# hamaadshah/gan_deeplearning4j

Hardware: NVIDIA H100
Metric: images/sec (full G+D step) (higher is better)
Workload: dtype bf16

## Files before the change

### gan_deeplearning4j_b200/csrc/kernels_ew.cu

```cuda
#include <stdlib.h>
#include <algorithm>
#include "kernels.h"
#include "common.cuh"

namespace b2g {

uint64_t g_launch_count = 0;
const char* g_ew_last_kernel = "";

template <typename T>
__global__ void nchw_f32_to_nhwc_kernel(const float* __restrict__ src, T* __restrict__ dst, int N, int C, int HW) { pdl_enter();
  size_t total = (size_t)N * C * HW;
  for (size_t i = blockIdx.x * (size_t)blockDim.x + threadIdx.x; i < total; i += (size_t)gridDim.x * blockDim.x) {
    int c = i % C; size_t t = i / C; int p = t % HW; size_t n = t / HW;
    stf(dst, i, src[(n * C + c) * HW + p]);
  }
}
template <typename T>
__global__ void nhwc_to_nchw_f32_kernel(const T* __restrict__ src, float* __restrict__ dst, int N, int C, int HW) { pdl_enter();
  size_t total = (size_t)N * C * HW;
  for (size_t i = blockIdx.x * (size_t)blockDim.x + threadIdx.x; i < total; i += (size_t)gridDim.x * blockDim.x) {
    int p = i % HW; size_t t = i / HW; int c = t % C; size_t n = t / C;
    dst[i] = ldf(src, (n * HW + p) * C + c);
  }
}
template <typename T>
__global__ void permute_kernel(const T* __restrict__ src, T* __restrict__ dst, int N, int C, int HW, int to_nhwc) { pdl_enter();
  size_t total = (size_t)N * C * HW;
  for (size_t i = blockIdx.x * (size_t)blockDim.x + threadIdx.x; i < total; i += (size_t)gridDim.x * blockDim.x) {
    if (to_nhwc) { int c = i % C; size_t t = i / C; int p = t % HW; size_t n = t / HW; dst[i] = src[(n * C + c) * HW + p]; }
    else         { int p = i % HW; size_t t = i / HW; int c = t % C; size_t n = t / C; dst[i] = src[(n * HW + p) * C + c]; }
  }
}
#define DISPATCH_ACT(act, ACTC, ...)                                                            \
  switch (act) {                                                                                \
    case ACT_IDENTITY: { constexpr int ACTC = ACT_IDENTITY; __VA_ARGS__; } break;               \
    case ACT_RELU: { constexpr int ACTC = ACT_RELU; __VA_ARGS__; } break;                       \
    case ACT_LRELU: { constexpr int ACTC = ACT_LRELU; __VA_ARGS__; } break;                     \
    default: { constexpr int ACTC = -1; __VA_ARGS__; } break;                                   \
  }
int device_sm_count() {
  static int sms[64] = {}; int d = 0; cudaGetDevice(&d); if (d < 0 || d >= 64) d = 0;
  if (!sms[d]) { int v = 0; cudaDeviceGetAttribute(&v, cudaDevAttrMultiProcessorCount, d); sms[d] = v > 0 ? v : 1; }
  return sms[d];
}
static inline int vec4_blocks(size_t n_vec) { const size_t cap = (size_t)device_sm_count() * 4; size_t b = (n_vec + 1023) / 1024; if (b > cap) b = cap; if (b < 1) b = 1; return (int)b; }
static inline int ew_blocks(size_t n, int per = 256) { const size_t cap = (size_t)device_sm_count() * 16; size_t b = (n + per - 1) / per; if (b > cap) b = cap; if (b < 1) b = 1; return (int)b; }

void k_nchw_f32_to_nhwc(int prec, const float* src, void* dst, int N, int C, int HW, cudaStream_t s) {
  size_t n = (size_t)N * C * HW; if (!n) return;
  DISPATCH_PREC(prec, T, (launch_pdl(nchw_f32_to_nhwc_kernel<T>, dim3(ew_blocks(n)), dim3(256), (size_t)(0), s, src, (T*)dst, N, C, HW))); LAUNCHED();
}
void k_nhwc_to_nchw_f32(int prec, const void* src, float* dst, int N, int C, int HW, cudaStream_t s) {
  size_t n = (size_t)N * C * HW; if (!n) return;
  DISPATCH_PREC(prec, T, (launch_pdl(nhwc_to_nchw_f32_kernel<T>, dim3(ew_blocks(n)), dim3(256), (size_t)(0), s, (const T*)src, dst, N, C, HW))); LAUNCHED();
}
void k_permute(int prec, const void* src, void* dst, int N, int C, int HW, int to_nhwc, cudaStream_t s) {
  size_t n = (size_t)N * C * HW; if (!n) return;
  DISPATCH_PREC(prec, T, (launch_pdl(permute_kernel<T>, dim3(ew_blocks(n)), dim3(256), (size_t)(0), s, (const T*)src, (T*)dst, N, C, HW, to_nhwc))); LAUNCHED();
}
__global__ void cast_f32_to_bf16_kernel(const float* __restrict__ src, __nv_bfloat16* __restrict__ dst, size_t n) { pdl_enter();
  for (size_t i = blockIdx.x * (size_t)blockDim.x + threadIdx.x; i < n; i += (size_t)gridDim.x * blockDim.x) dst[i] = __float2bfloat16_rn(src[i]);
}
void k_cast_f32_to_bf16(const float* src, __nv_bfloat16* dst, size_t n, cudaStream_t s) {
  if (!n) return; launch_pdl(cast_f32_to_bf16_kernel, dim3(ew_blocks(n)), dim3(256), (size_t)(0), s, src, dst, n); LAUNCHED();
}
static const int SLICE_ELEMS = 1 << 20;
static inline int pick_slices(int rows, int C) {
  int cap = SLICE_ELEMS / (C > 0 ? C : 1); if (cap < 1) cap = 1; if (cap > 2048) cap = 2048;
  int S = rows / 8; if (S < 1) S = 1; if (S > cap) S = cap; return S;
}
size_t k_bn_scratch_floats(int C, int groups) { return (size_t)2 * groups * (SLICE_ELEMS + 2 * (size_t)C) + 64; }
size_t k_colsum_scratch_floats(int C) { return (size_t)(SLICE_ELEMS + C) + 64; }

__device__ __forceinline__ void unpack8(const uint4& u, float (&v)[8]) {
  const __nv_bfloat162* h = reinterpret_cast<const __nv_bfloat162*>(&u);
#pragma unroll
  for (int j = 0; j < 4; ++j) { float2 f = __bfloat1622float2(h[j]); v[2 * j] = f.x; v[2 * j + 1] = f.y; }
}
__device__ __forceinline__ uint4 pack8(const float (&v)[8]) {
  uint4 u; __nv_bfloat162* h = reinterpret_cast<__nv_bfloat162*>(&u);
#pragma unroll
  for (int j = 0; j < 4; ++j) h[j] = __floats2bfloat162_rn(v[2 * j], v[2 * j + 1]);
  return u;
}

template <typename T>
__global__ void bn_stats_partial_kernel(const T* __restrict__ x, int rows, int C, int S, float* __restrict__ psum, float* __restrict__ psq, float* __restrict__ pivot) { pdl_enter();
  int g = blockIdx.y;
  int idx = blockIdx.x * blockDim.x + threadIdx.x;
  if (idx >= S * C) return;
  int c = idx % C, sl = idx / C;
  const T* xg = x + (size_t)g * rows * C;
  const float k = ldf(xg, c);
  if (sl == 0) pivot[g * C + c] = k;
  float a = 0.f, b = 0.f;
  for (int r = sl; r < rows; r += S) { float v = ldf(xg, (size_t)r * C + c) - k; a += v; b = fmaf(v, v, b); }
  psum[((size_t)g * S + sl) * C + c] = a; psq[((size_t)g * S + sl) * C + c] = b;
}
static inline int vec_ty(int C) { int c8 = C / 8; int ty = 256 / c8; return ty < 1 ? 1 : ty; }
static inline bool vec_ok(int prec, int C) { return prec == PREC_BF16 && C % 8 == 0 && C / 8 <= 256 && 256 % (C / 8) == 0; }
static inline int vec_blocks(int rows, int C) { int ty = vec_ty(C); int b = rows / (ty * 4); int cap = SLICE_ELEMS / C; if (cap > 256) cap = 256; if (b > cap) b = cap; if (b < 1) b = 1; return b; }
template <int NV>
__device__ __forceinline__ void block_fold_write(float (&acc)[NV][8], int C, int C8, int c8, int ty, int TY, float* const (&dst)[NV], size_t row_off) {
  __shared__ float sred[NV][2048];
#pragma unroll
  for (int v = 0; v < NV; ++v)
#pragma unroll
    for (int j = 0; j < 8; ++j) sred[v][ty * C + c8 * 8 + j] = acc[v][j];
  __syncthreads();
  for (int c = threadIdx.x; c < C; c += blockDim.x) {
#pragma unroll
    for (int v = 0; v < NV; ++v) { float a = 0.f; for (int k = 0; k < TY; ++k) a += sred[v][k * C + c]; dst[v][row_off + c] = a; }
  }
}
__global__ void __launch_bounds__(1024) bn_stats_final_kernel(const float* __restrict__ psum, const float* __restrict__ psq, const float* __restrict__ pivot, int rows, int C, int S, int groups, float eps,
                                      float* __restrict__ mean, float* __restrict__ invstd,
                                      const float* __restrict__ run_mean, const float* __restrict__ run_var, float* g_mean, float* g_var, float decay) { pdl_enter();
  __shared__ double sa[32][33], sb[32][33];
  const int tx = threadIdx.x & 31, ty = threadIdx.x >> 5, c = blockIdx.x * 32 + tx;
  double acc_gm = 0.0, acc_gv = 0.0;
  for (int g = 0; g < groups; ++g) {
    double a = 0.0, b = 0.0;
    if (c < C) for (int sl0 = ty; sl0 < S; sl0 += 32 * 8) {
      float va[8], vb[8];
#pragma unroll
      for (int q = 0; q < 8; ++q) { const int sl = sl0 + 32 * q; va[q] = sl < S ? psum[((size_t)g * S + sl) * C + c] : 0.f; vb[q] = sl < S ? psq[((size_t)g * S + sl) * C + c] : 0.f; }
#pragma unroll
      for (int q = 0; q < 8; ++q) { a += va[q]; b += vb[q]; }
    }
    sa[ty][tx] = a; sb[ty][tx] = b;
    __syncthreads();
    if (ty == 0 && c < C) {
      for (int k = 1; k < 32; ++k) { a += sa[k][tx]; b += sb[k][tx]; }
      const double d = a / rows, mu = (double)pivot[g * C + c] + d; double var = b / rows - d * d; if (var < 0) var = 0;
      mean[g * C + c] = (float)mu; invstd[g * C + c] = (float)(1.0 / sqrt(var + (double)eps));
      if (g_mean) { acc_gm += (1.0 - decay) * ((double)run_mean[c] - mu); acc_gv += (1.0 - decay) * ((double)run_var[c] - var); }
    }
    __syncthreads();
  }
  if (g_mean && ty == 0 && c < C) { g_mean[c] = (float)(acc_gm / groups); g_var[c] = (float)(acc_gv / groups); }
}
void k_bn_stats(int prec, const void* x, int rows, int C, int groups, float* scratch, float* mean, float* invstd, float eps,
                const float* run_mean, const float* run_var, float* g_mean, float* g_var, float decay, cudaStream_t s) {
  const int S = pick_slices(rows, C);
  float* psum = scratch; float* psq = scratch + (size_t)groups * S * C; float* pivot = psq + (size_t)groups * S * C;
  dim3 grid((S * C + 255) / 256, groups);
  DISPATCH_PREC(prec, T, (launch_pdl(bn_stats_partial_kernel<T>, dim3(grid), dim3(256), (size_t)(0), s, (const T*)x, rows, C, S, psum, psq, pivot)));
  LAUNCHED();
  launch_pdl(bn_stats_final_kernel, dim3((C + 31) / 32), dim3(1024), (size_t)(0), s, psum, psq, (const float*)pivot, rows, C, S, groups, eps, mean, invstd, run_mean, run_var, g_mean, g_var, decay); LAUNCHED();
}
__global__ void bn_prep_infer_kernel(const float* __restrict__ rm, const float* __restrict__ rv, int C, int groups, float eps, float* mean, float* invstd) { pdl_enter();
  int i = blockIdx.x * blockDim.x + threadIdx.x; if (i >= C * groups) return;
  int c = i % C; mean[i] = rm[c]; invstd[i] = 1.0f / sqrtf(rv[c] + eps);
}
__global__ void bn_fold_kernel(const float* __restrict__ rm, const float* __restrict__ rv, const float* __restrict__ gamma, const float* __restrict__ beta, const float* __restrict__ cb, int C, float eps, float* scale, float* shift) { pdl_enter();
  int c = blockIdx.x * blockDim.x + threadIdx.x; if (c >= C) return;
  const float sc = gamma[c] / sqrtf(rv[c] + eps); scale[c] = sc; shift[c] = beta[c] - rm[c] * sc + (cb ? cb[c] * sc : 0.f);
}
void k_bn_fold(const float* rm, const float* rv, const float* gamma, const float* beta, const float* cb, int C, float eps, float* scale, float* shift, cudaStream_t s) {
  launch_pdl(bn_fold_kernel, dim3((C + 255) / 256), dim3(256), (size_t)0, s, rm, rv, gamma, beta, cb, C, eps, scale, shift); LAUNCHED();
}
void k_bn_prep_infer(const float* run_mean, const float* run_var, int C, int groups, float eps, float* mean, float* invstd, cudaStream_t s) {
  launch_pdl(bn_prep_infer_kernel, dim3((C * groups + 255) / 256), dim3(256), (size_t)(0), s, run_mean, run_var, C, groups, eps, mean, invstd); LAUNCHED();
}

template <typename T>
__global__ void bn_apply_kernel(const T* __restrict__ x, T* __restrict__ y, int rows, int C, int groups, const float* __restrict__ mean,
                                const float* __restrict__ invstd, const float* __restrict__ gamma, const float* __restrict__ beta, int act, float alpha) { pdl_enter();
  size_t per_group = (size_t)rows * C, total = per_group * groups;
  for (size_t i = blockIdx.x * (size_t)blockDim.x + threadIdx.x; i < total; i += (size_t)gridDim.x * blockDim.x) {
    int c = i % C; int g = i / per_group;
    float v = (ldf(x, i) - mean[g * C + c]) * invstd[g * C + c];
    stf(y, i, act_fwd(act, fmaf(gamma[c], v, beta[c]), alpha));
  }
}
template <int ACTC>
__global__ void __launch_bounds__(256, 3) bn_apply_bf16x8_kernel(const uint4* __restrict__ x, uint4* __restrict__ y, int rows, int C, int groups, const float* __restrict__ mean,
                                       const float* __restrict__ invstd, const float* __restrict__ gamma, const float* __restrict__ beta, int act, float alpha) { pdl_enter();
  const int C8 = C / 8; const size_t per_group = (size_t)rows * C8;
  const size_t t0 = blockIdx.x * (size_t)blockDim.x + threadIdx.x, stride = (size_t)gridDim.x * blockDim.x;
  const int c0 = (int)(t0 % C8) * 8;
  for (int g = 0; g < groups; ++g) {
    float mu[8], is[8], ga[8], be[8];
#pragma unroll
    for (int j = 0; j < 8; ++j) { mu[j] = mean[g * C + c0 + j]; is[j] = invstd[g * C + c0 + j]; ga[j] = gamma[c0 + j]; be[j] = beta[c0 + j]; }
    const uint4* xg = x + g * per_group; uint4* yg = y + g * per_group;
    for (size_t i = t0; i < per_group; i += 4 * stride) {
      uint4 xa[4];
#pragma unroll
      for (int q = 0; q < 4; ++q) if (i + q * stride < per_group) xa[q] = xg[i + q * stride];
#pragma unroll
      for (int q = 0; q < 4; ++q) if (i + q * stride < per_group) {
        float v[8]; unpack8(xa[q], v);
#pragma unroll
        for (int j = 0; j < 8; ++j) v[j] = act_fwd(ACTC < 0 ? act : ACTC, fmaf(ga[j], (v[j] - mu[j]) * is[j], be[j]), alpha);
        yg[i + q * stride] = pack8(v);
      }
    }
  }
}
void k_bn_apply(int prec, const void* x, void* y, int rows, int C, int groups, const float* mean, const float* invstd,
                const float* gamma, const float* beta, int act, float alpha, cudaStream_t s) {
  size_t n = (size_t)rows * C * groups; if (!n) return;
  if (vec_ok(prec, C)) {
    DISPATCH_ACT(act, ACTC, launch_pdl(bn_apply_bf16x8_kernel<ACTC>, dim3(vec4_blocks((size_t)rows * C / 8)), dim3(256), (size_t)(0), s, (const uint4*)x, (uint4*)y, rows, C, groups, mean, invstd, gamma, beta, act, alpha));
  } else {
    DISPATCH_PREC(prec, T, (launch_pdl(bn_apply_kernel<T>, dim3(ew_blocks(n)), dim3(256), (size_t)(0), s, (const T*)x, (T*)y, rows, C, groups, mean, invstd, gamma, beta, act, alpha)));
  }
  LAUNCHED();
}

template <typename T>
__global__ void bn_bwd_partial_kernel(const T* __restrict__ x, const T* __restrict__ eo, int rows, int C, int S, const float* __restrict__ mean,
                                      const float* __restrict__ invstd, const float* __restrict__ gamma, const float* __restrict__ beta, int act, float alpha,
                                      float* __restrict__ p1, float* __restrict__ p2) { pdl_enter();
  int g = blockIdx.y;
  int idx = blockIdx.x * blockDim.x + threadIdx.x;
  if (idx >= S * C) return;
  int c = idx % C, sl = idx / C;
  const T* xg = x + (size_t)g * rows * C; const T* eg = eo + (size_t)g * rows * C;
  float mu = mean[g * C + c], is = invstd[g * C + c], ga = gamma[c], be = beta[c];
  float a = 0.f, b = 0.f;
  for (int r = sl; r < rows; r += S) {
    float xh = (ldf(xg, (size_t)r * C + c) - mu) * is;
    float dy = ldf(eg, (size_t)r * C + c) * act_grad_from_pre(act, fmaf(ga, xh, be), alpha);
    a += dy; b = fmaf(dy, xh, b);
  }
  p1[((size_t)g * S + sl) * C + c] = a; p2[((size_t)g * S + sl) * C + c] = b;
}
__global__ void __launch_bounds__(1024) bn_bwd_final_kernel(const float* __restrict__ p1, const float* __restrict__ p2, int rows, int C, int S, int groups,
                                    float* __restrict__ c1, float* __restrict__ c2, float* g_gamma, float* g_beta, int want) { pdl_enter();
  __shared__ double sa[32][33], sb[32][33];
  const int tx = threadIdx.x & 31, ty = threadIdx.x >> 5, c = blockIdx.x * 32 + tx;
  double tg = 0.0, tb = 0.0;
  for (int g = 0; g < groups; ++g) {
    double a = 0.0, b = 0.0;
    if (c < C) for (int sl0 = ty; sl0 < S; sl0 += 32 * 8) {
      float va[8], vb[8];
#pragma unroll
      for (int q = 0; q < 8; ++q) { const int sl = sl0 + 32 * q; va[q] = sl < S ? p1[((size_t)g * S + sl) * C + c] : 0.f; vb[q] = sl < S ? p2[((size_t)g * S + sl) * C + c] : 0.f; }
#pragma unroll
      for (int q = 0; q < 8; ++q) { a += va[q]; b += vb[q]; }
    }
    sa[ty][tx] = a; sb[ty][tx] = b;
    __syncthreads();
    if (ty == 0 && c < C) {
      for (int k = 1; k < 32; ++k) { a += sa[k][tx]; b += sb[k][tx]; }
      c1[g * C + c] = (float)(a / rows); c2[g * C + c] = (float)(b / rows); tb += a; tg += b;
    }
    __syncthreads();
  }
  if (want && ty == 0 && c < C) { g_beta[c] += (float)tb; g_gamma[c] += (float)tg; }
}
template <typename T>
__global__ void bn_bwd_apply_kernel(const T* __restrict__ x, const T* __restrict__ eo, T* __restrict__ ei, int rows, int C, int groups,
                                    const float* __restrict__ mean, const float* __restrict__ invstd, const float* __restrict__ gamma,
                                    const float* __restrict__ beta, int act, float alpha, const float* __restrict__ c1, const float* __restrict__ c2) { pdl_enter();
  size_t per_group = (size_t)rows * C, total = per_group * groups;
  for (size_t i = blockIdx.x * (size_t)blockDim.x + threadIdx.x; i < total; i += (size_t)gridDim.x * blockDim.x) {
    int c = i % C; int g = i / per_group; int k = g * C + c;
    float xh = (ldf(x, i) - mean[k]) * invstd[k];
    float dy = ldf(eo, i) * act_grad_from_pre(act, fmaf(gamma[c], xh, beta[c]), alpha);
    stf(ei, i, gamma[c] * invstd[k] * (dy - c1[k] - xh * c2[k]));
  }
}
void k_bn_bwd(int prec, const void* x, const void* eps_out, void* eps_in, int rows, int C, int groups,
              const float* mean, const float* invstd, const float* gamma, const float* beta, int act, float alpha,
              float* scratch, float* g_gamma, float* g_beta, int want, cudaStream_t s) {
  const int S = pick_slices(rows, C);
  float* p1 = scratch; float* p2 = p1 + (size_t)groups * S * C; float* c1 = p2 + (size_t)groups * S * C; float* c2 = c1 + (size_t)groups * C;
  dim3 grid((S * C + 255) / 256, groups);
  DISPATCH_PREC(prec, T, (launch_pdl(bn_bwd_partial_kernel<T>, dim3(grid), dim3(256), (size_t)(0), s, (const T*)x, (const T*)eps_out, rows, C, S, mean, invstd, gamma, beta, act, alpha, p1, p2)));
  LAUNCHED();
  launch_pdl(bn_bwd_final_kernel, dim3((C + 31) / 32), dim3(1024), (size_t)(0), s, p1, p2, rows, C, S, groups, c1, c2, g_gamma, g_beta, want); LAUNCHED();
  if (eps_in) {
    size_t n = (size_t)rows * C * groups;
    DISPATCH_PREC(prec, T, (launch_pdl(bn_bwd_apply_kernel<T>, dim3(ew_blocks(n)), dim3(256), (size_t)(0), s, (const T*)x, (const T*)eps_out, (T*)eps_in, rows, C, groups, mean, invstd, gamma, beta, act, alpha, c1, c2)));
    LAUNCHED();
  }
}


bool k_bn_vec_ok(int prec, int C) { return vec_ok(prec, C); }
size_t k_bn_acc_elems(int C, int groups) { return (size_t)groups * 4 * C; }

template <int NV, typename A>
__device__ __forceinline__ void block_fold_acc(A (&acc)[NV][8], int C, int c8, int ty, int TY, unsigned long long* accbase ) {
  __shared__ double sred[NV][2048];
#pragma unroll
  for (int v = 0; v < NV; ++v)
#pragma unroll
    for (int j = 0; j < 8; ++j) sred[v][ty * C + c8 * 8 + j] = acc[v][j];
  __syncthreads();
  for (int c = threadIdx.x; c < C; c += blockDim.x) {
#pragma unroll
    for (int v = 0; v < NV; ++v) { double a = 0.0; for (int k = 0; k < TY; ++k) a += sred[v][k * C + c]; sacc_add(accbase + (size_t)v * 2 * C, (size_t)C, (size_t)c, a); }
  }
}
__global__ void __launch_bounds__(256) bn_stats_acc_kernel(const uint4* __restrict__ x, int rows, int C, int S, unsigned long long* __restrict__ accp) { pdl_enter();
  const int g = blockIdx.y, C8 = C / 8, TY = 256 / C8, c8 = threadIdx.x % C8, ty = threadIdx.x / C8, sl = blockIdx.x;
  const int chunk = (rows + S - 1) / S, r0 = sl * chunk, r1 = min(rows, r0 + chunk);
  const uint4* xg = x + (size_t)g * rows * C8;
  double acc[2][8];
#pragma unroll
  for (int j = 0; j < 8; ++j) { acc[0][j] = 0.0; acc[1][j] = 0.0; }
#pragma unroll 4
  for (int r = r0 + ty; r < r1; r += TY) { float v[8]; unpack8(xg[(size_t)r * C8 + c8], v);
#pragma unroll
    for (int j = 0; j < 8; ++j) { acc[0][j] += v[j]; acc[1][j] = fma((double)v[j], (double)v[j], acc[1][j]); } }
  block_fold_acc<2>(acc, C, c8, ty, TY, accp + (size_t)g * 4 * C);
}
void k_bn_stats_acc(const void* x, int rows, int C, int groups, unsigned long long* acc, cudaStream_t s) {
  const int S = vec_blocks(rows, C);
  launch_pdl(bn_stats_acc_kernel, dim3(S, groups), dim3(256), (size_t)0, s, (const uint4*)x, rows, C, S, acc); LAUNCHED();
}

__device__ __forceinline__ float bn_pre_act(int act, float x, float sc, float be, float mu) {
  return (act == ACT_RELU || act == ACT_LRELU) ? fmaf(x, sc, fmaf(-mu, sc, be)) : fmaf(x - mu, sc, be);
}
template <int ACTC>
__global__ void __launch_bounds__(256, 3) bn_apply_acc_kernel(const uint4* __restrict__ x, uint4* __restrict__ y, int rows, int C, int groups, const unsigned long long* __restrict__ accp,
                                                             const float* __restrict__ gamma, const float* __restrict__ beta, int act, float alpha, float eps, float* __restrict__ coef,
                                                             const float* __restrict__ run_mean, const float* __restrict__ run_var, float* g_mean, float* g_var, float decay, int replicas) { pdl_enter();
  extern __shared__ float s_cf[];
  const double cnt = (double)rows * replicas, inv_cnt = 1.0 / cnt;
  const bool writer = blockIdx.x == 0;
  const int C8 = C / 8; const size_t per_group = (size_t)rows * C8;
  const size_t t0 = blockIdx.x * (size_t)blockDim.x + threadIdx.x, stride = (size_t)gridDim.x * blockDim.x;
  uint4 xa[4];
#pragma unroll
  for (int q = 0; q < 4; ++q) if (t0 + q * stride < per_group) xa[q] = x[t0 + q * stride];
  for (int c = threadIdx.x; c < C; c += blockDim.x) {
    double agm = 0.0, agv = 0.0;
    for (int g = 0; g < groups; ++g) {
      const unsigned long long* a = accp + (size_t)g * 4 * C;
      const double mu = sacc_read(a, (size_t)C, (size_t)c) * inv_cnt; double var = sacc_read(a + 2 * (size_t)C, (size_t)C, (size_t)c) * inv_cnt - mu * mu; if (var < 0) var = 0;
      const float is = (float)(1.0 / sqrt(var + (double)eps)), sc = gamma[c] * is, sh = fmaf(-(float)mu, sc, beta[c]);
      s_cf[(g * 2 + 0) * C + c] = sc; s_cf[(g * 2 + 1) * C + c] = sh;
      if (writer) {
        coef[(size_t)(g * 4 + 0) * C + c] = sc; coef[(size_t)(g * 4 + 1) * C + c] = beta[c]; coef[(size_t)(g * 4 + 2) * C + c] = (float)mu; coef[(size_t)(g * 4 + 3) * C + c] = is;
        if (g_mean) { agm += (1.0 - decay) * ((double)run_mean[c] - mu); agv += (1.0 - decay) * ((double)run_var[c] - var); }
      }
    }
    if (writer && g_mean) { g_mean[c] = (float)(agm / groups); g_var[c] = (float)(agv / groups); }
  }
  __syncthreads();
  const int c0 = (int)(t0 % C8) * 8;
  bool preloaded = true;
  for (int g = 0; g < groups; ++g) {
    float sc[8], sh[8];
#pragma unroll
    for (int j = 0; j < 8; ++j) { sc[j] = s_cf[(g * 2 + 0) * C + c0 + j]; sh[j] = s_cf[(g * 2 + 1) * C + c0 + j]; }
    const uint4* xg = x + g * per_group; uint4* yg = y + g * per_group;
    for (size_t i = t0; i < per_group; i += 4 * stride) {
      if (!preloaded) {
#pragma unroll
        for (int q = 0; q < 4; ++q) if (i + q * stride < per_group) xa[q] = xg[i + q * stride];
      }
      preloaded = false;
#pragma unroll
      for (int q = 0; q < 4; ++q) if (i + q * stride < per_group) {
        float v[8]; unpack8(xa[q], v);
#pragma unroll
        for (int j = 0; j < 8; ++j) v[j] = act_fwd(ACTC < 0 ? act : ACTC, fmaf(v[j], sc[j], sh[j]), alpha);
        yg[i + q * stride] = pack8(v);
      }
    }
  }
}
void k_bn_apply_acc(const void* x, void* y, int rows, int C, int groups, const unsigned long long* acc, const float* gamma, const float* beta, int act, float alpha, float eps,
                    float* coef, const float* run_mean, const float* run_var, float* g_mean, float* g_var, float decay, cudaStream_t s, int replicas) {
  const size_t smem = sizeof(float) * 2 * groups * C;
  DISPATCH_ACT(act, ACTC, launch_pdl(bn_apply_acc_kernel<ACTC>, dim3(vec4_blocks((size_t)rows * C / 8)), dim3(256), smem, s, (const uint4*)x, (uint4*)y, rows, C, groups, acc, gamma, beta, act, alpha, eps,
                                     coef, run_mean, run_var, g_mean, g_var, decay, replicas));
  LAUNCHED();
}

template <int ACTC>
__global__ void __launch_bounds__(256, 3) bn_bwd_stats_acc_kernel(const uint4* __restrict__ x, const uint4* __restrict__ eo, int rows, int C, int S, const float* __restrict__ coef,
                                                                 int act, float alpha, unsigned long long* __restrict__ accp) { pdl_enter();
  const int g = blockIdx.y, C8 = C / 8, TY = 256 / C8, c8 = threadIdx.x % C8, ty = threadIdx.x / C8, sl = blockIdx.x;
  const int chunk = (rows + S - 1) / S, r0 = sl * chunk, r1 = min(rows, r0 + chunk);
  const uint4* xg = x + (size_t)g * rows * C8; const uint4* eg = eo + (size_t)g * rows * C8;
  float sc[8], be[8], mu[8], is[8], acc[2][8];
#pragma unroll
  for (int j = 0; j < 8; ++j) { const int c = c8 * 8 + j; sc[j] = coef[(size_t)(g * 4 + 0) * C + c]; be[j] = coef[(size_t)(g * 4 + 1) * C + c]; mu[j] = coef[(size_t)(g * 4 + 2) * C + c]; is[j] = coef[(size_t)(g * 4 + 3) * C + c]; acc[0][j] = 0.f; acc[1][j] = 0.f; }
#pragma unroll 4
  for (int r = r0 + ty; r < r1; r += TY) {
    float xv[8], ev[8]; unpack8(xg[(size_t)r * C8 + c8], xv); unpack8(eg[(size_t)r * C8 + c8], ev);
#pragma unroll
    for (int j = 0; j < 8; ++j) { const float xh = (xv[j] - mu[j]) * is[j]; const float dy = ev[j] * act_grad_from_pre(ACTC < 0 ? act : ACTC, bn_pre_act(ACTC < 0 ? act : ACTC, xv[j], sc[j], be[j], mu[j]), alpha); acc[0][j] += dy; acc[1][j] = fmaf(dy, xh, acc[1][j]); }
  }
  block_fold_acc<2>(acc, C, c8, ty, TY, accp + (size_t)g * 4 * C);
}
void k_bn_bwd_stats_acc(const void* x, const void* eps_out, int rows, int C, int groups, const float* coef, int act, float alpha, unsigned long long* acc, cudaStream_t s) {
  const int S = vec_blocks(rows, C);
  DISPATCH_ACT(act, ACTC, launch_pdl(bn_bwd_stats_acc_kernel<ACTC>, dim3(S, groups), dim3(256), (size_t)0, s, (const uint4*)x, (const uint4*)eps_out, rows, C, S, coef, act, alpha, acc));
  LAUNCHED();
}

template <int ACTC, bool PREMUL>
__global__ void __launch_bounds__(256, 2) bn_bwd_apply_acc_kernel(const uint4* __restrict__ x, const uint4* __restrict__ eo, uint4* __restrict__ ei, int rows, int C, int groups,
                                                                 const float* __restrict__ coef, int act, float alpha, const unsigned long long* __restrict__ accp,
                                                                 float* g_gamma, float* g_beta, int want, int replicas) { pdl_enter();
  extern __shared__ float s_k[];
  const double cnt = (double)rows * replicas, inv_cnt = 1.0 / cnt;
  const bool writer = blockIdx.x == 0 && want;
  const int C8 = C / 8; const size_t per_group = (size_t)rows * C8;
  const size_t t0 = blockIdx.x * (size_t)blockDim.x + threadIdx.x, stride = (size_t)gridDim.x * blockDim.x;
  uint4 xa[4], ea[4];
  if (ei) {
#pragma unroll
    for (int q = 0; q < 4; ++q) if (t0 + q * stride < per_group) { xa[q] = x[t0 + q * stride]; ea[q] = eo[t0 + q * stride]; }
  }
  for (int c = threadIdx.x; c < C; c += blockDim.x) {
    double tb = 0.0, tg = 0.0;
    for (int g = 0; g < groups; ++g) {
      const unsigned long long* a = accp + (size_t)g * 4 * C;
      const double s1 = sacc_read(a, (size_t)C, (size_t)c); double s2 = sacc_read(a + 2 * (size_t)C, (size_t)C, (size_t)c);
      if (PREMUL) s2 = (double)coef[(size_t)(g * 4 + 3) * C + c] * (s2 - (double)coef[(size_t)(g * 4 + 2) * C + c] * s1);
      s_k[(g * 2 + 0) * C + c] = (float)(s1 * inv_cnt); s_k[(g * 2 + 1) * C + c] = (float)(s2 * inv_cnt); tb += s1; tg += s2;
    }
    if (writer) { g_beta[c] += (float)(tb / replicas); g_gamma[c] += (float)(tg / replicas); }
  }
  __syncthreads();
  if (!ei) return;
  const int c0 = (int)(t0 % C8) * 8;
  bool preloaded = true;
  for (int g = 0; g < groups; ++g) {
    float sc[8], be[8], mu[8], is[8], k1[8], k2[8];
#pragma unroll
    for (int j = 0; j < 8; ++j) { const int c = c0 + j; sc[j] = coef[(size_t)(g * 4 + 0) * C + c]; be[j] = coef[(size_t)(g * 4 + 1) * C + c]; mu[j] = coef[(size_t)(g * 4 + 2) * C + c]; is[j] = coef[(size_t)(g * 4 + 3) * C + c];
      k1[j] = s_k[(g * 2 + 0) * C + c]; k2[j] = s_k[(g * 2 + 1) * C + c]; }
    const uint4* xg = x + g * per_group; const uint4* eg = eo + g * per_group; uint4* ig = ei + g * per_group;
    for (size_t i = t0; i < per_group; i += 4 * stride) {
      if (!preloaded) {
#pragma unroll
        for (int q = 0; q < 4; ++q) if (i + q * stride < per_group) { xa[q] = xg[i + q * stride]; ea[q] = eg[i + q * stride]; }
      }
      preloaded = false;
#pragma unroll
      for (int q = 0; q < 4; ++q) if (i + q * stride < per_group) {
        float xv[8], ev[8], o[8]; unpack8(xa[q], xv); unpack8(ea[q], ev);
#pragma unroll
        for (int j = 0; j < 8; ++j) { const float xh = (xv[j] - mu[j]) * is[j];
          const float dy = PREMUL ? ev[j] : ev[j] * act_grad_from_pre(ACTC < 0 ? act : ACTC, bn_pre_act(ACTC < 0 ? act : ACTC, xv[j], sc[j], be[j], mu[j]), alpha); o[j] = sc[j] * (dy - k1[j] - xh * k2[j]); }
        ig[i + q * stride] = pack8(o);
      }
    }
  }
}
void k_bn_bwd_apply_acc(const void* x, const void* eps_out, void* eps_in, int rows, int C, int groups, const float* coef, int act, float alpha, int premul,
                        const unsigned long long* acc, float* g_gamma, float* g_beta, int want, cudaStream_t s, int replicas) {
  const size_t smem = sizeof(float) * 2 * groups * C;
  const dim3 grid(eps_in ? vec4_blocks((size_t)rows * C / 8) : 1);
  if (premul) { launch_pdl(bn_bwd_apply_acc_kernel<ACT_IDENTITY, true>, grid, dim3(256), smem, s, (const uint4*)x, (const uint4*)eps_out, (uint4*)eps_in, rows, C, groups, coef, act, alpha, acc, g_gamma, g_beta, want, replicas); }
  else { DISPATCH_ACT(act, ACTC, launch_pdl(bn_bwd_apply_acc_kernel<ACTC, false>, grid, dim3(256), smem, s, (const uint4*)x, (const uint4*)eps_out, (uint4*)eps_in, rows, C, groups, coef, act, alpha, acc, g_gamma, g_beta, want, replicas)); }
  LAUNCHED();
}


__device__ __forceinline__ void st_release_sys(unsigned* p, unsigned v) { asm volatile("st.release.sys.global.u32 [%0], %1;" ::"l"(p), "r"(v) : "memory"); }
__device__ __forceinline__ unsigned ld_acquire_sys(const unsigned* p) { unsigned v; asm volatile("ld.acquire.sys.global.u32 %0, [%1];" : "=r"(v) : "l"(p) : "memory"); return v; }
__device__ __forceinline__ void p2p_wait_all(const unsigned* flags, int world, unsigned e) {
  for (int r = 0; r < world; ++r) {
    unsigned it = 0;
    while ((int)(ld_acquire_sys(flags + r) - e) < 0) { if (++it > (1u << 27)) __trap(); __nanosleep(32); }
  }
}
__global__ void __launch_bounds__(512) p2p_allreduce_kernel(const P2pArgs a) {
  __shared__ unsigned s_e;
  if (threadIdx.x == 0) s_e = *reinterpret_cast<volatile unsigned*>(a.state) + 1;
  __syncthreads();
  const unsigned e = s_e; const int W = a.world;
  unsigned* mine = a.flags[a.rank];
  if (blockIdx.x == 0 && threadIdx.x < W) st_release_sys(a.flags[threadIdx.x] + a.rank, e);
  if (threadIdx.x == 0) p2p_wait_all(mine, W, e);
  __syncthreads();
  const size_t nv = a.n / 4, chunk = (nv + W - 1) / W, v0 = min(nv, (size_t)a.rank * chunk), v1 = min(nv, v0 + chunk);
  for (size_t i = v0 + blockIdx.x * (size_t)blockDim.x + threadIdx.x; i < v1; i += (size_t)gridDim.x * blockDim.x) {
    float4 acc = __ldcg(reinterpret_cast<const float4*>(a.grads[0]) + i);
    for (int r = 1; r < W; ++r) { const float4 v = __ldcg(reinterpret_cast<const float4*>(a.grads[r]) + i); acc.x += v.x; acc.y += v.y; acc.z += v.z; acc.w += v.w; }
    for (int r = 0; r < W; ++r) __stcg(reinterpret_cast<float4*>(a.grads[r]) + i, acc);
  }
  if (a.rank == W - 1 && blockIdx.x == 0 && threadIdx.x < (a.n & 3)) {
    const size_t i = nv * 4 + threadIdx.x; float acc = __ldcg(a.grads[0] + i);
    for (int r = 1; r < W; ++r) acc += __ldcg(a.grads[r] + i);
    for (int r = 0; r < W; ++r) __stcg(a.grads[r] + i, acc);
  }
  __threadfence_system();
  __syncthreads();
  if (threadIdx.x == 0) {
    const unsigned t = atomicAdd(a.state + 1, 1u);
    if (t == gridDim.x - 1) {
      a.state[1] = 0;
      for (int r = 0; r < W; ++r) st_release_sys(a.flags[r] + 8 + a.rank, e);
      p2p_wait_all(mine + 8, W, e);
      *reinterpret_cast<volatile unsigned*>(a.state) = e;
      __threadfence();
    }
  }
}
void k_p2p_allreduce(const P2pArgs& a, cudaStream_t s) {
  const size_t slice = (a.n / 4 + a.world - 1) / a.world;
  int blocks = (int)((slice + 2047) / 2048); if (blocks > 120) blocks = 120; if (blocks < 1) blocks = 1;
  p2p_allreduce_kernel<<<blocks, 512, 0, s>>>(a); LAUNCHED();
}

template <typename T>
__global__ void act_fwd_kernel(const T* __restrict__ x, T* __restrict__ y, size_t n, int act, float alpha) { pdl_enter();
  for (size_t i = blockIdx.x * (size_t)blockDim.x + threadIdx.x; i < n; i += (size_t)gridDim.x * blockDim.x) stf(y, i, act_fwd(act, ldf(x, i), alpha));
}
template <typename T>
__global__ void act_bwd_out_kernel(const T* __restrict__ a, const T* __restrict__ eo, T* __restrict__ ei, size_t n, int act, float alpha) { pdl_enter();
  for (size_t i = blockIdx.x * (size_t)blockDim.x + threadIdx.x; i < n; i += (size_t)gridDim.x * blockDim.x)
    stf(ei, i, ldf(eo, i) * act_grad_from_out(act, ldf(a, i), alpha));
}
void k_act_fwd(int prec, const void* x, void* y, size_t n, int act, float alpha, cudaStream_t s) {
  if (!n) return; DISPATCH_PREC(prec, T, (launch_pdl(act_fwd_kernel<T>, dim3(ew_blocks(n)), dim3(256), (size_t)(0), s, (const T*)x, (T*)y, n, act, alpha))); LAUNCHED();
  g_ew_last_kernel = "act_fwd_kernel";
}
template <int ACTC>
__global__ void __launch_bounds__(256, 4) act_bwd_out_bf16x8_kernel(const uint4* __restrict__ a, const uint4* __restrict__ eo, uint4* __restrict__ ei, size_t n8, int act, float alpha) { pdl_enter();
  const size_t stride = (size_t)gridDim.x * blockDim.x;
  for (size_t i = blockIdx.x * (size_t)blockDim.x + threadIdx.x; i < n8; i += 4 * stride) {
    uint4 aa[4], ea[4];
#pragma unroll
    for (int q = 0; q < 4; ++q) if (i + q * stride < n8) { aa[q] = a[i + q * stride]; ea[q] = eo[i + q * stride]; }
#pragma unroll
    for (int q = 0; q < 4; ++q) if (i + q * stride < n8) {
      float av[8], ev[8], o[8]; unpack8(aa[q], av); unpack8(ea[q], ev);
#pragma unroll
      for (int j = 0; j < 8; ++j) o[j] = ev[j] * act_grad_from_out(ACTC < 0 ? act : ACTC, av[j], alpha);
      ei[i + q * stride] = pack8(o);
    }
  }
}
void k_act_bwd_from_output(int prec, const void* a, const void* eo, void* ei, size_t n, int act, float alpha, cudaStream_t s) {
  if (!n) return;
  if (prec == PREC_BF16 && n % 8 == 0 && ((reinterpret_cast<uintptr_t>(a) | reinterpret_cast<uintptr_t>(eo) | reinterpret_cast<uintptr_t>(ei)) & 15) == 0) {
    DISPATCH_ACT(act, ACTC, launch_pdl(act_bwd_out_bf16x8_kernel<ACTC>, dim3(vec4_blocks(n / 8)), dim3(256), (size_t)0, s, (const uint4*)a, (const uint4*)eo, (uint4*)ei, n / 8, act, alpha)); LAUNCHED();
    g_ew_last_kernel = "act_bwd_out_bf16x8_kernel"; return;
  }
  DISPATCH_PREC(prec, T, (launch_pdl(act_bwd_out_kernel<T>, dim3(ew_blocks(n)), dim3(256), (size_t)(0), s, (const T*)a, (const T*)eo, (T*)ei, n, act, alpha))); LAUNCHED();
  g_ew_last_kernel = "act_bwd_out_kernel";
}
void k_sigmoid_out(int prec, const void* z, void* p, size_t n, cudaStream_t s) { k_act_fwd(prec, z, p, n, ACT_SIGMOID, 0.f, s); }

template <typename T>
__global__ void maxpool_fwd_kernel(const T* __restrict__ x, T* __restrict__ y, uint8_t* __restrict__ arg, int N, int H, int W, int C, int OH, int OW, int KH, int KW, int SH, int SW) { pdl_enter();
  size_t total = (size_t)N * OH * OW * C;
  for (size_t i = blockIdx.x * (size_t)blockDim.x + threadIdx.x; i < total; i += (size_t)gridDim.x * blockDim.x) {
    int c = i % C; size_t t = i / C; int ox = t % OW; t /= OW; int oy = t % OH; size_t n = t / OH;
    float best = -INFINITY; int bi = 0;
    for (int r = 0; r < KH; ++r) for (int q = 0; q < KW; ++q) {
      float v = ldf(x, ((n * H + oy * SH + r) * W + ox * SW + q) * C + c);
      if (v > best) { best = v; bi = r * KW + q; }
    }
    stf(y, i, best); arg[i] = (uint8_t)bi;
  }
}
template <typename T>
__global__ void maxpool_bwd_kernel(const T* __restrict__ eo, const uint8_t* __restrict__ arg, T* __restrict__ ei, int N, int H, int W, int C, int OH, int OW, int KH, int KW, int SH, int SW) { pdl_enter();
  size_t total = (size_t)N * H * W * C;
  for (size_t i = blockIdx.x * (size_t)blockDim.x + threadIdx.x; i < total; i += (size_t)gridDim.x * blockDim.x) {
    int c = i % C; size_t t = i / C; int ix = t % W; t /= W; int iy = t % H; size_t n = t / H;
    float acc = 0.f;
    for (int r = 0; r < KH; ++r) { int ty = iy - r; if (ty < 0 || ty % SH) continue; int oy = ty / SH; if (oy >= OH) continue;
      for (int q = 0; q < KW; ++q) { int tx = ix - q; if (tx < 0 || tx % SW) continue; int ox = tx / SW; if (ox >= OW) continue;
        size_t o = ((n * OH + oy) * OW + ox) * C + c;
        if (arg[o] == r * KW + q) acc += ldf(eo, o);
      } }
    stf(ei, i, acc);
  }
}
void k_maxpool_fwd(int prec, const void* x, void* y, uint8_t* arg, int N, int H, int W, int C, int OH, int OW, int KH, int KW, int SH, int SW, cudaStream_t s) {
  size_t n = (size_t)N * OH * OW * C; if (!n) return;
  DISPATCH_PREC(prec, T, (launch_pdl(maxpool_fwd_kernel<T>, dim3(ew_blocks(n)), dim3(256), (size_t)(0), s, (const T*)x, (T*)y, arg, N, H, W, C, OH, OW, KH, KW, SH, SW))); LAUNCHED();
  g_ew_last_kernel = "maxpool_fwd_kernel";
}
void k_maxpool_bwd(int prec, const void* eo, const uint8_t* arg, void* ei, int N, int H, int W, int C, int OH, int OW, int KH, int KW, int SH, int SW, cudaStream_t s) {
  size_t n = (size_t)N * H * W * C; if (!n) return;
  DISPATCH_PREC(prec, T, (launch_pdl(maxpool_bwd_kernel<T>, dim3(ew_blocks(n)), dim3(256), (size_t)(0), s, (const T*)eo, arg, (T*)ei, N, H, W, C, OH, OW, KH, KW, SH, SW))); LAUNCHED();
  g_ew_last_kernel = "maxpool_bwd_kernel";
}
template <typename T>
__global__ void upsample_fwd_kernel(const T* __restrict__ x, T* __restrict__ y, int N, int H, int W, int C, int f) { pdl_enter();
  size_t total = (size_t)N * H * f * W * f * C;
  for (size_t i = blockIdx.x * (size_t)blockDim.x + threadIdx.x; i < total; i += (size_t)gridDim.x * blockDim.x) {
    int c = i % C; size_t t = i / C; int ox = t % (W * f); t /= (W * f); int oy = t % (H * f); size_t n = t / (H * f);
    y[i] = x[((n * H + oy / f) * W + ox / f) * C + c];
  }
}
template <typename T>
__global__ void upsample_bwd_kernel(const T* __restrict__ eo, T* __restrict__ ei, int N, int H, int W, int C, int f) { pdl_enter();
  size_t total = (size_t)N * H * W * C;
  for (size_t i = blockIdx.x * (size_t)blockDim.x + threadIdx.x; i < total; i += (size_t)gridDim.x * blockDim.x) {
    int c = i % C; size_t t = i / C; int ix = t % W; t /= W; int iy = t % H; size_t n = t / H;
    float acc = 0.f;
    for (int a = 0; a < f; ++a) for (int b = 0; b < f; ++b) acc += ldf(eo, ((n * H * f + iy * f + a) * (size_t)(W * f) + ix * f + b) * C + c);
    stf(ei, i, acc);
  }
}
void k_upsample_fwd(int prec, const void* x, void* y, int N, int H, int W, int C, int f, cudaStream_t s) {
  size_t n = (size_t)N * H * f * W * f * C; if (!n) return;
  DISPATCH_PREC(prec, T, (launch_pdl(upsample_fwd_kernel<T>, dim3(ew_blocks(n)), dim3(256), (size_t)(0), s, (const T*)x, (T*)y, N, H, W, C, f))); LAUNCHED();
  g_ew_last_kernel = "upsample_fwd_kernel";
}
void k_upsample_bwd(int prec, const void* eo, void* ei, int N, int H, int W, int C, int f, cudaStream_t s) {
  size_t n = (size_t)N * H * W * C; if (!n) return;
  DISPATCH_PREC(prec, T, (launch_pdl(upsample_bwd_kernel<T>, dim3(ew_blocks(n)), dim3(256), (size_t)(0), s, (const T*)eo, (T*)ei, N, H, W, C, f))); LAUNCHED();
  g_ew_last_kernel = "upsample_bwd_kernel";
}

template <typename T>
__global__ void xent_kernel(const T* __restrict__ z, const float* __restrict__ y, T* __restrict__ dz, float* __restrict__ loss_sums, int rows, float clip) { pdl_enter();
  int g = blockIdx.x;
  __shared__ double red[32];
  double acc = 0.0;
  for (int r = threadIdx.x; r < rows; r += blockDim.x) {
    size_t i = (size_t)g * rows + r;
    float zi = ldf(z, i), yi = y[i], loss, grad;
    float sg = 1.0f / (1.0f + expf(-zi));
    if (clip > 0.f) {
      float p = fminf(fmaxf(sg, clip), 1.0f - clip);
      loss = -(yi * logf(p) + (1.0f - yi) * logf(1.0f - p));
      grad = (p - yi) / (p * (1.0f - p)) * sg * (1.0f - sg);
    } else {
      loss = fmaxf(zi, 0.f) + log1pf(expf(-fabsf(zi))) - yi * zi;
      grad = sg - yi;
    }
    acc += loss; stf(dz, i, grad);
  }
  for (int o = 16; o; o >>= 1) acc += __shfl_xor_sync(0xffffffffu, acc, o);
  if (threadIdx.x % 32 == 0) red[threadIdx.x / 32] = acc;
  __syncthreads();
  if (threadIdx.x == 0) { double t = 0; for (int w = 0; w < (blockDim.x + 31) / 32; ++w) t += red[w]; loss_sums[g] = (float)t; }
}
void k_xent(int prec, const void* z, const float* y, void* dz, float* loss_sums, int rows, int groups, float clip, cudaStream_t s) {
  DISPATCH_PREC(prec, T, (launch_pdl(xent_kernel<T>, dim3(groups), dim3(1024), (size_t)(0), s, (const T*)z, y, (T*)dz, loss_sums, rows, clip))); LAUNCHED();
  g_ew_last_kernel = "xent_kernel";
}

template <typename T>
__global__ void softmax_xent_kernel(const T* __restrict__ z, const float* __restrict__ y, T* __restrict__ dz, T* __restrict__ p_out, float* __restrict__ loss_sum, int rows, int K) { pdl_enter();
  __shared__ double red[32];
  double acc = 0.0;
  for (int r = threadIdx.x; r < rows; r += blockDim.x) {
    float m = -INFINITY; for (int k = 0; k < K; ++k) m = fmaxf(m, ldf(z, (size_t)r * K + k));
    float den = 0.f; for (int k = 0; k < K; ++k) den += expf(ldf(z, (size_t)r * K + k) - m);
    for (int k = 0; k < K; ++k) {
      const float p = expf(ldf(z, (size_t)r * K + k) - m) / den;
      if (p_out) stf(p_out, (size_t)r * K + k, p);
      if (dz) { const float yk = y[(size_t)r * K + k]; stf(dz, (size_t)r * K + k, p - yk); acc -= (double)yk * log((double)fminf(fmaxf(p, 1e-10f), 1.0f - 1e-10f)); }
    }
  }
  for (int o = 16; o; o >>= 1) acc += __shfl_xor_sync(0xffffffffu, acc, o);
  if (threadIdx.x % 32 == 0) red[threadIdx.x / 32] = acc;
  __syncthreads();
  if (threadIdx.x == 0 && loss_sum) { double t = 0; for (int w = 0; w < (blockDim.x + 31) / 32; ++w) t += red[w]; loss_sum[0] = (float)t; }
}
void k_softmax_xent(int prec, const void* z, const float* y, void* dz, void* p_out, float* loss_sums, int rows, int K, cudaStream_t s) {
  DISPATCH_PREC(prec, T, (launch_pdl(softmax_xent_kernel<T>, dim3(1), dim3(1024), (size_t)0, s, (const T*)z, y, (T*)dz, (T*)p_out, loss_sums, rows, K))); LAUNCHED();
  g_ew_last_kernel = "softmax_xent_kernel";
}

constexpr int LOSS_THREADS = 256, LOSS_ELEMS_PER_BLOCK = 1024, LOSS_MAX_GRID = 1024;
int k_loss_blocks(size_t n_per_group, int groups) {
  const size_t b = (n_per_group + LOSS_ELEMS_PER_BLOCK - 1) / LOSS_ELEMS_PER_BLOCK;
  return (int)std::min<size_t>(std::max<size_t>(b, 1), std::max(1, LOSS_MAX_GRID / groups));
}
template <typename T>
__global__ void __launch_bounds__(LOSS_THREADS) loss_kernel(const T* __restrict__ z, const float* __restrict__ y, T* __restrict__ dz, float* __restrict__ loss_sums,
                                                           size_t n_per_group, int n_out, int bpg, int loss, int act, float alpha, double* partial, unsigned* ticket) {
  pdl_enter();
  __shared__ double red[LOSS_THREADS / 32];
  __shared__ int last;
  const int g = blockIdx.x / bpg, b = blockIdx.x % bpg;
  const float nf = (float)n_out;
  double acc = 0.0;
  for (size_t j = (size_t)b * LOSS_THREADS + threadIdx.x; j < n_per_group; j += (size_t)bpg * LOSS_THREADS) {
    const size_t i = (size_t)g * n_per_group + j;
    const float a = act_fwd(act, ldf(z, i), alpha), yi = y[i];
    const double e = (double)a - (double)yi, m = 1.0 - (double)yi * (double)a;
    double l; float ga;
    switch (loss) {
      case LOSS_MSE: l = e * e; ga = 2.0f * (a - yi) / nf; break;
      case LOSS_L2: l = e * e; ga = 2.0f * (a - yi); break;
      case LOSS_L1: l = fabs(e); ga = (float)((a > yi) - (a < yi)); break;
      case LOSS_MAE: l = fabs(e); ga = (float)((a > yi) - (a < yi)) / nf; break;
      case LOSS_HINGE: l = fmax(m, 0.0); ga = m > 0.0 ? -yi : 0.f; break;
      case LOSS_SQUARED_HINGE: l = m > 0.0 ? m * m : 0.0; ga = m > 0.0 ? -2.0f * yi * (float)m : 0.f; break;
      default: l = (double)yi * (double)a; ga = yi / nf; break;
    }
    acc += l;
    stf(dz, i, ga * act_grad_from_out(act, a, alpha));
  }
  const double tot = block_sum(acc, red);
  if (threadIdx.x == 0) {
    partial[blockIdx.x] = tot;
    __threadfence();
    last = atomicAdd(ticket, 1u) == gridDim.x - 1;
  }
  __syncthreads();
  if (!last) return;
  __threadfence();
  const bool per_out = loss == LOSS_MSE || loss == LOSS_MAE || loss == LOSS_WASSERSTEIN;
  const int warp = threadIdx.x >> 5, lane = threadIdx.x & 31;
  for (int gg = warp; gg < (int)(gridDim.x / bpg); gg += LOSS_THREADS / 32) {
    double s = 0.0;
    for (int k = lane; k < bpg; k += 32) s += __ldcg(partial + (size_t)gg * bpg + k);
#pragma unroll
    for (int o = 16; o > 0; o >>= 1) s += __shfl_xor_sync(0xffffffffu, s, o);
    if (lane == 0) loss_sums[gg] = (float)(per_out ? s / n_out : s);
  }
  if (threadIdx.x == 0) { *ticket = 0u; __threadfence(); }
}
void k_loss(int prec, int loss, int act, float alpha, const void* z, const float* y, void* dz, float* loss_sums, int rows_per_group, int n_out, int groups,
            double* partial, unsigned* ticket, cudaStream_t s) {
  const size_t n = (size_t)rows_per_group * n_out; const int bpg = k_loss_blocks(n, groups);
  DISPATCH_PREC(prec, T, (launch_pdl(loss_kernel<T>, dim3(groups * bpg), dim3(LOSS_THREADS), (size_t)0, s, (const T*)z, y, (T*)dz, loss_sums, n, n_out, bpg,
                                     loss, act, alpha, partial, ticket))); LAUNCHED();
  g_ew_last_kernel = "loss_kernel";
}

template <typename T>
__global__ void colsum_partial_kernel(const T* __restrict__ x, int rows, int C, int S, float* __restrict__ p) { pdl_enter();
  int idx = blockIdx.x * blockDim.x + threadIdx.x; if (idx >= S * C) return;
  int c = idx % C, sl = idx / C; float a = 0.f;
  for (int r = sl; r < rows; r += S) a += ldf(x, (size_t)r * C + c);
  p[(size_t)sl * C + c] = a;
}
__global__ void __launch_bounds__(256) colsum_partial_bf16x8_kernel(const uint4* __restrict__ x, int rows, int C, int S, float* __restrict__ p) { pdl_enter();
  const int C8 = C / 8, TY = 256 / C8, c8 = threadIdx.x % C8, ty = threadIdx.x / C8, sl = blockIdx.x;
  const int chunk = (rows + S - 1) / S, r0 = sl * chunk, r1 = min(rows, r0 + chunk);
  float acc[1][8];
#pragma unroll
  for (int j = 0; j < 8; ++j) acc[0][j] = 0.f;
  for (int r = r0 + ty; r < r1; r += TY) { float v[8]; unpack8(x[(size_t)r * C8 + c8], v);
#pragma unroll
    for (int j = 0; j < 8; ++j) acc[0][j] += v[j]; }
  float* const dst[1] = {p};
  block_fold_write<1>(acc, C, C8, c8, ty, TY, dst, (size_t)sl * C);
}
__global__ void __launch_bounds__(512) colsum_final_kernel(const float* __restrict__ p, int C, int S, float* out, int accumulate) { pdl_enter();
  __shared__ double sa[16][33];
  const int tx = threadIdx.x & 31, ty = threadIdx.x >> 5, c = blockIdx.x * 32 + tx;
  double a = 0.0;
  if (c < C) for (int sl0 = ty; sl0 < S; sl0 += 16 * 8) {
    float va[8];
#pragma unroll
    for (int q = 0; q < 8; ++q) { const int sl = sl0 + 16 * q; va[q] = sl < S ? p[(size_t)sl * C + c] : 0.f; }
#pragma unroll
    for (int q = 0; q < 8; ++q) a += va[q];
  }
  sa[ty][tx] = a;
  __syncthreads();
  if (ty == 0 && c < C) { for (int k = 1; k < 16; ++k) a += sa[k][tx]; out[c] = (accumulate ? out[c] : 0.f) + (float)a; }
}
template <int C>
// ... 275 lines not shown
```

Measured before the change: 91990.

## Double-buffer BN apply loads and size grids to resident occupancy

The BN forward-apply and backward-apply kernels now prefetch the next batch of vectors, including the first batch of the next group, while the current batch is computed. This replaces the load-then-compute pattern. Grid size is now capped at the number of blocks that can be resident at once, found with an occupancy query and cached per device. The backward batch drops to 2 vectors per tensor to limit register pressure. The added prefetch buffers may raise register use, and a smaller grid means each thread runs more loop iterations.

```diff
diff --git a/gan_deeplearning4j_b200/csrc/kernels_ew.cu b/gan_deeplearning4j_b200/csrc/kernels_ew.cu
--- a/gan_deeplearning4j_b200/csrc/kernels_ew.cu
+++ b/gan_deeplearning4j_b200/csrc/kernels_ew.cu
@@ -319,6 +319,21 @@
 __device__ __forceinline__ float bn_pre_act(int act, float x, float sc, float be, float mu) {
   return (act == ACT_RELU || act == ACT_LRELU) ? fmaf(x, sc, fmaf(-mu, sc, be)) : fmaf(x - mu, sc, be);
 }
+static const int BN_BATCH = 4, BN_BWD_BATCH = 2;
+template <int NQ>
+__device__ __forceinline__ void bn_load_batch(const uint4* __restrict__ src, size_t i, size_t stride, size_t n, uint4 (&buf)[NQ]) {
+#pragma unroll
+  for (int q = 0; q < NQ; ++q) if (i + q * stride < n) buf[q] = src[i + q * stride];
+}
+template <auto KERN>
+static int resident_blocks(size_t smem) {
+  static int blocks[64] = {}; int d = 0; cudaGetDevice(&d); if (d < 0 || d >= 64) d = 0;
+  if (!blocks[d]) { int per_sm = 0; cudaOccupancyMaxActiveBlocksPerMultiprocessor(&per_sm, KERN, 256, smem); blocks[d] = std::max(1, per_sm) * device_sm_count(); }
+  return blocks[d];
+}
+static inline int bn_stream_blocks(size_t n_vec, int batch, int resident) {
+  const size_t b = (n_vec + 256 * batch - 1) / (256 * batch); return (int)std::max<size_t>(1, std::min<size_t>(b, (size_t)resident));
+}
 template <int ACTC>
 __global__ void __launch_bounds__(256, 3) bn_apply_acc_kernel(const uint4* __restrict__ x, uint4* __restrict__ y, int rows, int C, int groups, const unsigned long long* __restrict__ accp,
                                                              const float* __restrict__ gamma, const float* __restrict__ beta, int act, float alpha, float eps, float* __restrict__ coef,
@@ -328,9 +343,8 @@
   const bool writer = blockIdx.x == 0;
   const int C8 = C / 8; const size_t per_group = (size_t)rows * C8;
   const size_t t0 = blockIdx.x * (size_t)blockDim.x + threadIdx.x, stride = (size_t)gridDim.x * blockDim.x;
-  uint4 xa[4];
-#pragma unroll
-  for (int q = 0; q < 4; ++q) if (t0 + q * stride < per_group) xa[q] = x[t0 + q * stride];
+  uint4 xa[BN_BATCH];
+  bn_load_batch(x, t0, stride, per_group, xa);
   for (int c = threadIdx.x; c < C; c += blockDim.x) {
     double agm = 0.0, agv = 0.0;
     for (int g = 0; g < groups; ++g) {
@@ -347,33 +361,32 @@
   }
   __syncthreads();
   const int c0 = (int)(t0 % C8) * 8;
-  bool preloaded = true;
   for (int g = 0; g < groups; ++g) {
     float sc[8], sh[8];
 #pragma unroll
     for (int j = 0; j < 8; ++j) { sc[j] = s_cf[(g * 2 + 0) * C + c0 + j]; sh[j] = s_cf[(g * 2 + 1) * C + c0 + j]; }
     const uint4* xg = x + g * per_group; uint4* yg = y + g * per_group;
-    for (size_t i = t0; i < per_group; i += 4 * stride) {
-      if (!preloaded) {
-#pragma unroll
-        for (int q = 0; q < 4; ++q) if (i + q * stride < per_group) xa[q] = xg[i + q * stride];
-      }
-      preloaded = false;
-#pragma unroll
-      for (int q = 0; q < 4; ++q) if (i + q * stride < per_group) {
+    for (size_t i = t0; i < per_group; i += BN_BATCH * stride) {
+      uint4 xb[BN_BATCH];
+      if (i + BN_BATCH * stride < per_group) bn_load_batch(xg, i + BN_BATCH * stride, stride, per_group, xb);
+      else if (g + 1 < groups) bn_load_batch(xg + per_group, t0, stride, per_group, xb);
+#pragma unroll
+      for (int q = 0; q < BN_BATCH; ++q) if (i + q * stride < per_group) {
         float v[8]; unpack8(xa[q], v);
 #pragma unroll
         for (int j = 0; j < 8; ++j) v[j] = act_fwd(ACTC < 0 ? act : ACTC, fmaf(v[j], sc[j], sh[j]), alpha);
         yg[i + q * stride] = pack8(v);
       }
+#pragma unroll
+      for (int q = 0; q < BN_BATCH; ++q) xa[q] = xb[q];
     }
   }
 }
 void k_bn_apply_acc(const void* x, void* y, int rows, int C, int groups, const unsigned long long* acc, const float* gamma, const float* beta, int act, float alpha, float eps,
                     float* coef, const float* run_mean, const float* run_var, float* g_mean, float* g_var, float decay, cudaStream_t s, int replicas) {
-  const size_t smem = sizeof(float) * 2 * groups * C;
-  DISPATCH_ACT(act, ACTC, launch_pdl(bn_apply_acc_kernel<ACTC>, dim3(vec4_blocks((size_t)rows * C / 8)), dim3(256), smem, s, (const uint4*)x, (uint4*)y, rows, C, groups, acc, gamma, beta, act, alpha, eps,
-                                     coef, run_mean, run_var, g_mean, g_var, decay, replicas));
+  const size_t smem = sizeof(float) * 2 * groups * C, n_vec = (size_t)rows * C / 8;
+  DISPATCH_ACT(act, ACTC, launch_pdl(bn_apply_acc_kernel<ACTC>, dim3(bn_stream_blocks(n_vec, BN_BATCH, resident_blocks<bn_apply_acc_kernel<ACTC>>(smem))), dim3(256), smem, s,
+                                     (const uint4*)x, (uint4*)y, rows, C, groups, acc, gamma, beta, act, alpha, eps, coef, run_mean, run_var, g_mean, g_var, decay, replicas));
   LAUNCHED();
 }
 
@@ -409,11 +422,8 @@
   const bool writer = blockIdx.x == 0 && want;
   const int C8 = C / 8; const size_t per_group = (size_t)rows * C8;
   const size_t t0 = blockIdx.x * (size_t)blockDim.x + threadIdx.x, stride = (size_t)gridDim.x * blockDim.x;
-  uint4 xa[4], ea[4];
-  if (ei) {
-#pragma unroll
-    for (int q = 0; q < 4; ++q) if (t0 + q * stride < per_group) { xa[q] = x[t0 + q * stride]; ea[q] = eo[t0 + q * stride]; }
-  }
+  uint4 xa[BN_BWD_BATCH], ea[BN_BWD_BATCH];
+  if (ei) { bn_load_batch(x, t0, stride, per_group, xa); bn_load_batch(eo, t0, stride, per_group, ea); }
   for (int c = threadIdx.x; c < C; c += blockDim.x) {
     double tb = 0.0, tg = 0.0;
     for (int g = 0; g < groups; ++g) {
@@ -427,36 +437,39 @@
   __syncthreads();
   if (!ei) return;
   const int c0 = (int)(t0 % C8) * 8;
-  bool preloaded = true;
   for (int g = 0; g < groups; ++g) {
     float sc[8], be[8], mu[8], is[8], k1[8], k2[8];
 #pragma unroll
     for (int j = 0; j < 8; ++j) { const int c = c0 + j; sc[j] = coef[(size_t)(g * 4 + 0) * C + c]; be[j] = coef[(size_t)(g * 4 + 1) * C + c]; mu[j] = coef[(size_t)(g * 4 + 2) * C + c]; is[j] = coef[(size_t)(g * 4 + 3) * C + c];
       k1[j] = s_k[(g * 2 + 0) * C + c]; k2[j] = s_k[(g * 2 + 1) * C + c]; }
     const uint4* xg = x + g * per_group; const uint4* eg = eo + g * per_group; uint4* ig = ei + g * per_group;
-    for (size_t i = t0; i < per_group; i += 4 * stride) {
-      if (!preloaded) {
-#pragma unroll
-        for (int q = 0; q < 4; ++q) if (i + q * stride < per_group) { xa[q] = xg[i + q * stride]; ea[q] = eg[i + q * stride]; }
-      }
-      preloaded = false;
-#pragma unroll
-      for (int q = 0; q < 4; ++q) if (i + q * stride < per_group) {
+    for (size_t i = t0; i < per_group; i += BN_BWD_BATCH * stride) {
+      uint4 xb[BN_BWD_BATCH], eb[BN_BWD_BATCH];
+      if (i + BN_BWD_BATCH * stride < per_group) { bn_load_batch(xg, i + BN_BWD_BATCH * stride, stride, per_group, xb); bn_load_batch(eg, i + BN_BWD_BATCH * stride, stride, per_group, eb); }
+      else if (g + 1 < groups) { bn_load_batch(xg + per_group, t0, stride, per_group, xb); bn_load_batch(eg + per_group, t0, stride, per_group, eb); }
+#pragma unroll
+      for (int q = 0; q < BN_BWD_BATCH; ++q) if (i + q * stride < per_group) {
         float xv[8], ev[8], o[8]; unpack8(xa[q], xv); unpack8(ea[q], ev);
 #pragma unroll
         for (int j = 0; j < 8; ++j) { const float xh = (xv[j] - mu[j]) * is[j];
           const float dy = PREMUL ? ev[j] : ev[j] * act_grad_from_pre(ACTC < 0 ? act : ACTC, bn_pre_act(ACTC < 0 ? act : ACTC, xv[j], sc[j], be[j], mu[j]), alpha); o[j] = sc[j] * (dy - k1[j] - xh * k2[j]); }
         ig[i + q * stride] = pack8(o);
       }
+#pragma unroll
+      for (int q = 0; q < BN_BWD_BATCH; ++q) { xa[q] = xb[q]; ea[q] = eb[q]; }
     }
   }
 }
 void k_bn_bwd_apply_acc(const void* x, const void* eps_out, void* eps_in, int rows, int C, int groups, const float* coef, int act, float alpha, int premul,
                         const unsigned long long* acc, float* g_gamma, float* g_beta, int want, cudaStream_t s, int replicas) {
-  const size_t smem = sizeof(float) * 2 * groups * C;
-  const dim3 grid(eps_in ? vec4_blocks((size_t)rows * C / 8) : 1);
-  if (premul) { launch_pdl(bn_bwd_apply_acc_kernel<ACT_IDENTITY, true>, grid, dim3(256), smem, s, (const uint4*)x, (const uint4*)eps_out, (uint4*)eps_in, rows, C, groups, coef, act, alpha, acc, g_gamma, g_beta, want, replicas); }
-  else { DISPATCH_ACT(act, ACTC, launch_pdl(bn_bwd_apply_acc_kernel<ACTC, false>, grid, dim3(256), smem, s, (const uint4*)x, (const uint4*)eps_out, (uint4*)eps_in, rows, C, groups, coef, act, alpha, acc, g_gamma, g_beta, want, replicas)); }
+  const size_t smem = sizeof(float) * 2 * groups * C, n_vec = (size_t)rows * C / 8;
+  if (premul) {
+    const dim3 grid(eps_in ? bn_stream_blocks(n_vec, BN_BWD_BATCH, resident_blocks<bn_bwd_apply_acc_kernel<ACT_IDENTITY, true>>(smem)) : 1);
+    launch_pdl(bn_bwd_apply_acc_kernel<ACT_IDENTITY, true>, grid, dim3(256), smem, s, (const uint4*)x, (const uint4*)eps_out, (uint4*)eps_in, rows, C, groups, coef, act, alpha, acc, g_gamma, g_beta, want, replicas);
+  } else {
+    DISPATCH_ACT(act, ACTC, const dim3 grid(eps_in ? bn_stream_blocks(n_vec, BN_BWD_BATCH, resident_blocks<bn_bwd_apply_acc_kernel<ACTC, false>>(smem)) : 1);
+                 launch_pdl(bn_bwd_apply_acc_kernel<ACTC, false>, grid, dim3(256), smem, s, (const uint4*)x, (const uint4*)eps_out, (uint4*)eps_in, rows, C, groups, coef, act, alpha, acc, g_gamma, g_beta, want, replicas));
+  }
   LAUNCHED();
 }
 
```

Measured after the change: 92270, median of 6. No clear change (+0.3%).
